# psweens/VAN-GAN

Hardware: AMD Instinct MI355X
Metric: train Mvoxels/s (VanGan.train_step, 128^3 bf16) (higher is better)
Workload: dtype bf16; 1 GPU; VanGan.train_step, 128x128x128 volumes, batch 1 per GPU (global 1), clDice on, disc noise+dropout on; parallelism=dp1

## Files before the change

### van_gan_amd/csrc/vg_conv_thin.hip

```cpp
#include "vg_conv_common.h"
#include <stdio.h>

static int vg_ablate_knob(const char* key) {
    const int v = vg_tune(key, 0);
#ifdef VG_DEBUG_ABLATE
    return v;
#else
    if (v != 0) { fprintf(stderr, "libvangan_hip: VG_%s=%d is a timing-ablation knob of a -DVG_DEBUG_ABLATE build; this library refuses it\n", key, v); return -1; }
    return 0;
#endif
}
#include "vg_dma_common.h"
#include <type_traits>
#include <algorithm>
#include <cstdio>

#ifndef VG_THIN_WPE
#define VG_THIN_WPE 2
#endif
#ifndef VG_THIN_PF2
#define VG_THIN_PF2 0
#endif
#ifndef VG_THIN_PD
#define VG_THIN_PD 1
// ... 547 lines not shown
        auto epilogue = [&](auto masked_tag, const int pn16) {
            constexpr bool MASKED = decltype(masked_tag)::value;
            const bool dw_ok = !MASKED || (od < p.OD && ow < p.OW);
            const int nrow = MASKED ? p.OH - oh0 : TH;
            typedef __attribute__((ext_vector_type(2))) unsigned u32x2;
            typedef __attribute__((ext_vector_type(4))) unsigned u32x4;
#pragma unroll
            for (int q = 0; q < NP; ++q) {
            T* const optr = (T*)p.out + obase + cst + 16 * q + pn16;
            const T* const rptr = RES ? (const T*)p.res + obase + co0 + 16 * q : nullptr;
            const float* const r1ptr = RES ? (const float*)p.res + (((size_t)(n * p.BD + od + p.ood) * p.BH + oh0 + p.ooh) * p.BW + ow + p.oow) : nullptr;
            f32x2 eb[2], ers[2], erb[2];
            if constexpr (NP == 1) { eb[0] = e_b[0][0]; eb[1] = e_b[0][1]; if (RES) { ers[0] = e_rs[0][0]; ers[1] = e_rs[0][1]; erb[0] = e_rb[0][0]; erb[1] = e_rb[0][1]; } }
            else {
                const float* eq = ebs + 4 * kg + 16 * q;
                if (BIAS) { const f32x4 t = *(const f32x4*)eq; eb[0] = (f32x2){t[0], t[1]}; eb[1] = (f32x2){t[2], t[3]}; }
                if (RES) {
                    const f32x4 t = *(const f32x4*)(eq + 16 * NP), u = *(const f32x4*)(eq + 32 * NP);
                    ers[0] = (f32x2){t[0], t[1]}; ers[1] = (f32x2){t[2], t[3]}; erb[0] = (f32x2){u[0], u[1]}; erb[1] = (f32x2){u[2], u[3]};
                }
            }
            bf16x4 bx[BSTAT ? 8 : 1];
            f32x2 b_sc[2], b_sf[2], b_rs[2], b_nm[2];
            if (BSTAT) {
                constexpr int CW = 16 * NP * PL;
                const float* bq = bsc + 4 * kg + 16 * q + pn16;
                const f32x4 c_sc = *(const f32x4*)bq, c_sf = *(const f32x4*)(bq + CW), c_rs = *(const f32x4*)(bq + 2 * CW), c_nm = *(const f32x4*)(bq + 3 * CW);
                b_sc[0] = (f32x2){c_sc[0], c_sc[1]}; b_sc[1] = (f32x2){c_sc[2], c_sc[3]}; b_sf[0] = (f32x2){c_sf[0], c_sf[1]}; b_sf[1] = (f32x2){c_sf[2], c_sf[3]};
                b_rs[0] = (f32x2){c_rs[0], c_rs[1]}; b_rs[1] = (f32x2){c_rs[2], c_rs[3]};
                b_nm[0] = (f32x2){c_nm[0], c_nm[1]}; b_nm[1] = (f32x2){c_nm[2], c_nm[3]};
                auto fold = [&](int qq, int nn) { int i = qq - p.bs_pad; i = i < 0 ? -i : i; i = i >= nn ? 2 * nn - 2 - i : i; return min(max(i, 0), nn - 1); };
                const int XH = p.bs_H >> b_sh[q], XW = p.bs_W >> b_sh[q];
                const int id = fold(od + p.ood, p.bs_D) >> b_sh[q], iw = fold(ow + p.oow, p.bs_W) >> b_sh[q];
                const T* xcol = b_x[q] + ((size_t)id * XH * XW + iw) * b_cs[q];
#pragma unroll
                for (int j = 0; j < 8; ++j) {
                    if constexpr (NP == 1) bx[j] = bxp[j];
                    else {
                        const int ih = fold(oh0 + j + p.ooh, p.bs_H) >> b_sh[q];
                        bx[j] = *(const __attribute__((address_space(1))) bf16x4*)(uintptr_t)(xcol + (size_t)ih * XW * b_cs[q]);
                    }
                }
            }
            constexpr int RRN = NP == 1 ? 8 : 4;
            bf16x4 rr[RES ? 8 : 1];
#pragma unroll
            for (int jp = 0; jp < 8; jp += 2) {
                if constexpr (RES) {
                    if (jp % RRN == 0) {
#pragma unroll
                        for (int j = jp; j < jp + RRN; ++j) {
                            const bool ok = !MASKED || (dw_ok && j < nrow);
                            if (NP == 1 && p.res1) {
                                const float xv = ld_global(ok ? r1ptr + (size_t)j * p.BW : r1ptr);
                                rr[j] = __builtin_bit_cast(bf16x4, (u32x2){__float_as_uint(xv), 0u});
                            } else
                            rr[j] = *(const __attribute__((address_space(1))) bf16x4*)(uintptr_t)(ok ? rptr + j * rowpitch : rptr);
                        }
                    }
                }
                bf16x4 pk[2];
#pragma unroll
                for (int e = 0; e < 2; ++e) {
                    const int j = jp + e;
                    const bool ok = !MASKED || (dw_ok && j < nrow);
                    f32x2 v0 = {acc[q][j][0], acc[q][j][1]}, v1 = {acc[q][j][2], acc[q][j][3]};
                    if (BIAS) { v0 += eb[0]; v1 += eb[1]; }
                    if (RES) {
                        const bf16x4 r = rr[RES ? j : 0];
                        f32x2 r0 = {bf2f((bf16_t)r[0]), bf2f((bf16_t)r[1])}, r1 = {bf2f((bf16_t)r[2]), bf2f((bf16_t)r[3])};
                        if (NP == 1 && p.res1) { const float xv = __uint_as_float(__builtin_bit_cast(u32x2, r)[0]); r0 = (f32x2){xv, xv}; r1 = r0; }
                        v0 += r0 * ers[0] + erb[0]; v1 += r1 * ers[1] + erb[1];
                    }
                    pk[e] = (bf16x4){(short)f2bf(v0[0]), (short)f2bf(v0[1]), (short)f2bf(v1[0]), (short)f2bf(v1[1])};
                    if (STATS) {
                        f32x2 q0 = {bf2f((bf16_t)pk[e][0]), bf2f((bf16_t)pk[e][1])}, q1 = {bf2f((bf16_t)pk[e][2]), bf2f((bf16_t)pk[e][3])};
                        if (MASKED && !ok) { q0 = (f32x2){0.f, 0.f}; q1 = q0; }
                        f32x2 a0 = {s1[q][0], s1[q][1]}, a1 = {s1[q][2], s1[q][3]}, c0 = {s2[q][0], s2[q][1]}, c1 = {s2[q][2], s2[q][3]};
                        a0 += q0; a1 += q1; c0 += q0 * q0; c1 += q1 * q1;
                        s1[q][0] = a0[0]; s1[q][1] = a0[1]; s1[q][2] = a1[0]; s1[q][3] = a1[1]; s2[q][0] = c0[0]; s2[q][1] = c0[1]; s2[q][2] = c1[0]; s2[q][3] = c1[1];
                    }
                    if (BSTAT) {
                        f32x2 q0 = {bf2f((bf16_t)pk[e][0]), bf2f((bf16_t)pk[e][1])}, q1 = {bf2f((bf16_t)pk[e][2]), bf2f((bf16_t)pk[e][3])};
                        if (MASKED && !ok) { q0 = (f32x2){0.f, 0.f}; q1 = q0; }
                        const bf16x4 xr = bx[BSTAT ? j : 0];
                        const f32x2 x0 = {bf2f((bf16_t)xr[0]), bf2f((bf16_t)xr[1])}, x1 = {bf2f((bf16_t)xr[2]), bf2f((bf16_t)xr[3])};
                        const f32x2 pre0 = x0 * b_sc[0] + b_sf[0], pre1 = x1 * b_sc[1] + b_sf[1];
                        const f32x2 d0 = {pre0[0] > 0.f ? 1.f : b_slope, pre0[1] > 0.f ? 1.f : b_slope};
                        const f32x2 d1 = {pre1[0] > 0.f ? 1.f : b_slope, pre1[1] > 0.f ? 1.f : b_slope};
                        const f32x2 dn0 = q0 * d0, dn1 = q1 * d1;
                        const f32x2 xh0 = x0 * b_rs[0] + b_nm[0], xh1 = x1 * b_rs[1] + b_nm[1];
                        f32x2 a0 = {s1[q][0], s1[q][1]}, a1 = {s1[q][2], s1[q][3]}, c0 = {s2[q][0], s2[q][1]}, c1 = {s2[q][2], s2[q][3]};
                        a0 += dn0; a1 += dn1; c0 += dn0 * xh0; c1 += dn1 * xh1;
                        s1[q][0] = a0[0]; s1[q][1] = a0[1]; s1[q][2] = a1[0]; s1[q][3] = a1[1]; s2[q][0] = c0[0]; s2[q][1] = c0[1]; s2[q][2] = c1[0]; s2[q][3] = c1[1];
                    }
                }
                const u32x2 wa = __builtin_bit_cast(u32x2, pk[0]), wb2 = __builtin_bit_cast(u32x2, pk[1]);
                const u32x2 x0 = __builtin_amdgcn_permlane16_swap(wa[0], wb2[0], false, false);
                const u32x2 x1 = __builtin_amdgcn_permlane16_swap(wa[1], wb2[1], false, false);
                const u32x4 outv = {x0[0], x1[0], x0[1], x1[1]};
                const int j = jp + jodd;
                if (!MASKED || (dw_ok && j < nrow)) *(u32x4*)(optr + j * rowpitch) = outv;
                if constexpr (BSTAT && PL > 1) { __builtin_amdgcn_sched_barrier(0); bxn[jp] = bx_row(jp); bxn[jp + 1] = bx_row(jp + 1); __builtin_amdgcn_sched_barrier(0); }
            }
            }
        };
        if constexpr (PL == 1) { if (full) epilogue(std::false_type{}, 0); else epilogue(std::true_type{}, 0); }
        else {
            if (it) lds_only_barrier();
            if constexpr (BSTAT) {
                if (it == 0) {
                    bx_prepare(0, od0, oh0, ow0);
#pragma unroll
                    for (int j = 0; j < 8; ++j) bxn[j] = bx_row(j);
                }
            }
            if (!(p.dbg & 16) || it == 0) {
            thin_issue<MODE>(g, utab, tabat(od0, oh0, ow0), n, 0, tid, raw);
            thin_commit<MODE>(g, halo, scs, utab, tabat(od0, oh0, ow0), 0, tid, raw);
            }
#pragma unroll 1
            for (int pn = 0; pn < PL; ++pn) {
                const int use = it * PL + pn;
                if (use == 0) asm volatile("s_waitcnt vmcnt(0)" ::: "memory");
                lds_only_barrier();
                if (pn + 1 < PL || more) dma_weights(pn + 1 < PL ? pn + 1 : 0, (use + 1) & 1);
#pragma unroll
                for (int j = 0; j < 8; ++j) acc[0][j] = (f32x4){0.f, 0.f, 0.f, 0.f};
                if (!(p.dbg & 4)) mfma_panel(wlds + (use & 1) * WBUF + wbase);
                __builtin_amdgcn_s_waitcnt(0x0F70);
                asm volatile("" ::: "memory");
                if constexpr (BSTAT) {
#pragma unroll
                    for (int j = 0; j < 8; ++j) asm volatile("v_mov_b64 %0, %1" : "=&v"(bxp[j]) : "v"(bxn[j]));
                    if (pn + 1 < PL) bx_prepare(16 * (pn + 1), od0, oh0, ow0); else if (more) bx_prepare(0, ti_d * TD, ti_h * TH, ti_w * TW);
                }
                if (full) epilogue(std::false_type{}, 16 * pn); else epilogue(std::true_type{}, 16 * pn);
                if constexpr (BSTAT) {
#pragma unroll
                    for (int r = 0; r < 4; ++r) {
                        const float a = s1[0][r], b = s2[0][r];
#pragma unroll
                        for (int q = 0; q + 1 < PL; ++q) { s1[q][r] = s1[q + 1][r]; s2[q][r] = s2[q + 1][r]; }
                        s1[PL - 1][r] = a; s2[PL - 1][r] = b;
                    }
                }
            }
        }
    }
    if constexpr (PL > 1) asm volatile("s_waitcnt vmcnt(0)" ::: "memory");
    if ((STATS || BSTAT) && p.sums) {
#pragma unroll
        for (int q = 0; q < NP * PL; ++q)
#pragma unroll
            for (int r = 0; r < 4; ++r) {
                float a = s1[q][r], b = s2[q][r];
#pragma unroll
                for (int o = 1; o < 16; o <<= 1) { a += __shfl_xor(a, o); b += __shfl_xor(b, o); }
                if (li == 0) { atomicAdd(&stat[(16 * q + 4 * kg + r) * 2], a); atomicAdd(&stat[(16 * q + 4 * kg + r) * 2 + 1], b); }
            }
        __syncthreads();
        if (tid < 32 * NP * PL) {
            const int co = cop + (tid >> 1);
            const int stripe = blockIdx.x & (VG_STRIPES - 1);
            if (co < p.Cout) atomicAdd(&p.sums[(((size_t)stripe * gridDim.z + n) * p.Cout + co) * 2 + (tid & 1)], stat[tid]);
        }
        if constexpr (STATS && (NP == 2 || !RES)) { if (p.fin.ticket) vg_fin_tail(p.fin, p.sums, gridDim.z, p.Cout, gridDim.x * gridDim.y * gridDim.z, (int*)stat); }
    }
}

int vg_conv_thin_lds_bytes(const GatherIn& g, int np, int pl, bool up, bool wdma) {
    const int AL = (g.tiles_h * TH + 2) + (g.tiles_w * TW + 2) + (g.tiles_d * TD + 2);
    int head = HALO + (32 + 32 * np * pl + 64 * np * pl + (np > 1 ? 48 * np : 0) + 32) * 4 + (2 * HH * HW * 2 + 2 * AL) * 4;
    if (pl > 1 || wdma) return head + 1024 + 2 * 15 * 1024;
    if (up) {
        head += (g.tiles_h * (TH / 2) + 2 + g.tiles_d * (TD / 2) + 2 + 2 * UPCOLS + 16) * 4;
        return head + 16 + std::max(16 * np * (KCPAD * 2 + 16), 4 * 16 * np * WRSU);
    }
    return head + 16 + 16 * np * (KCPAD * 2 + 16);
}

bool vg_conv_thin_ok(const vg_conv_desc* d, const GatherIn& g, const ConvOut& k, const ConvCls& q, int np) {
    if (!vg_tune("CONV_THIN", 1)) return false;
    if (d->f32 || d->noise || q.ncls != 1 || d->istr != 1 || d->ostr != 1 || d->CK != 16 || d->ntaps != 27 || d->wpack) return false;
    if ((d->c_src0 + d->c_src1) % 16 || (d->Cout % (16 * np)) || d->tanh_out || d->accumulate || d->out_f32) return false;
    if (g.lean != VG_STAGE_PLAIN && g.lean != VG_STAGE_RELU) return false;
    if (!g.planar || g.HW != HW || g.HH != HH || g.HD != HD || g.HWp != HW || g.HHp != HH || g.DS != DSB || g.PSB != PSB) return false;
    if ((1 << g.twl) != TW || (1 << g.thl) != TH || (1 << g.tdl) != TD) return false;
    if (d->res && (d->bias == nullptr)) return false;
    if (d->res_c1 && np != 1) return false;
    if (k.Ktot != k.nchunks * KCPAD) return false;
    for (int i = 0; i < 27; ++i)
        if (d->tap_d[i] - g.tmin_d > 2 || d->tap_h[i] - g.tmin_h > 2 || d->tap_w[i] - g.tmin_w > 2) return false;
    if (np > 1) {
        const long wgs = (long)g.tiles_d * g.tiles_h * g.tiles_w * (d->Cout / (16 * np)) * d->N;
        if (!vg_tune("CONV_THIN2", 1) || wgs < vg_tune("CONV_THIN2_MINWG", 96)) return false;
    }
    return true;
}

template <int MODE, bool BIAS, bool RES, bool STATS, bool BSTAT, int NP, int PL = 1, bool UP = false>
static int launch_thin_np(const GatherIn& g, const ConvOut& k, int lds, hipStream_t s) {
    static bool attr_set = false;
    if (!attr_set) {
        (void)hipFuncSetAttribute((const void*)conv_thin_kernel<MODE, BIAS, RES, STATS, BSTAT, NP, PL, UP>, hipFuncAttributeMaxDynamicSharedMemorySize, VG_LDS_LIMIT);
        attr_set = true;
    }
    int per_cu = 2;
    if (lds > 0 && VG_LDS_LIMIT / lds < per_cu) per_cu = VG_LDS_LIMIT / lds;
    if (per_cu < 1) per_cu = 1;
    const int tiles = g.tiles_d * g.tiles_h * g.tiles_w;
    const int ny = k.Cout / (16 * NP * PL);
    const int wg = vg_tune("CONV_THIN_WGS", 0) > 0 ? vg_tune("CONV_THIN_WGS", 0) : 256 * per_cu;
    int bx = wg / (ny * g.N); if (bx < 1) bx = 1; if (bx > tiles) bx = tiles;
    ConvOut k2 = k; k2.xw = 0; k2.dbg = PL > 1 ? vg_ablate_knob("THIN_DBG") : 0;
    if (k2.dbg < 0) return VG_EINVAL;
    if (vg_tune("CONV_THIN_XCD", 1) && bx >= 16 && tiles >= 4 * bx) { bx &= ~7; k2.xw = 1; }
    char name[96];
    snprintf(name, sizeof name, "%s<m%%d,b%%d,r%%d,s%%d%s%s%s>|walk%%d|ch%%d", NP == 2 ? "conv_thin2" : "conv_thin", BSTAT ? (k.bs_x1 ? ",bs2" : ",bs1") : "", PL > 1 ? ",pl" : "", UP ? ",up" : "");
    if (vg_dry(name, MODE, (int)BIAS, (int)RES, (int)STATS, tiles > bx ? 1 : 0, k.nchunks > 1 ? (k.wdma ? 2 : 1) : 0)) return VG_OK;
    const bool fin_here = STATS && k2.fin.ticket && k2.sums && ((NP == 2 && vg_tune("CONV_THIN2_FIN", 1)) || (NP == 1 && !RES && vg_tune("CONV_THIN1_FIN", 1)));
    if (!fin_here) k2.fin.ticket = nullptr;
    if constexpr (!UP) k2.nup = 0;
    hipLaunchKernelGGL((conv_thin_kernel<MODE, BIAS, RES, STATS, BSTAT, NP, PL, UP>), dim3(bx, ny, g.N), dim3(256), lds, s, g, k2);
    if (fin_here) vg_fin_done = true;
    return vg_check_launch();
}
template <int MODE, bool BIAS, bool RES, bool STATS, bool BSTAT = false>
static int launch_thin(const GatherIn& g, const ConvOut& k, int np, hipStream_t s) {
    if constexpr (BSTAT && MODE == VG_STAGE_PLAIN) {
        const int lds3 = vg_conv_thin_lds_bytes(g, 1, 3);
        if (np == 1 && k.Cout == 48 && k.nchunks == 1 && 2 * lds3 <= VG_LDS_LIMIT && vg_tune("CONV_THIN_PL", 1))
            return launch_thin_np<MODE, BIAS, RES, STATS, BSTAT, 1, 3>(g, k, lds3, s);
    }
    if constexpr (MODE == VG_STAGE_RELU && BIAS && !RES && !BSTAT) {
        if (k.nup > 0 && k.nup < k.nchunks && vg_tune("CONV_THIN_UP", 0)) {
            const int ldsu = vg_conv_thin_lds_bytes(g, np, 1, true);
            if (2 * ldsu <= VG_LDS_LIMIT) {
                if (np == 1) return launch_thin_np<MODE, BIAS, RES, STATS, BSTAT, 1, 1, true>(g, k, ldsu, s);
            }
        }
    }
    if constexpr (MODE == VG_STAGE_RELU && !BSTAT) {
        const int ldsw = vg_conv_thin_lds_bytes(g, 1, 1, false, true);
        if (np == 1 && k.nchunks > 1 && 2 * ldsw <= VG_LDS_LIMIT && vg_tune("CONV_THIN_WDMA", 1)) {
            ConvOut kw = k; kw.wdma = 1;
            return launch_thin_np<MODE, BIAS, RES, STATS, BSTAT, 1>(g, kw, ldsw, s);
        }
    }
    const int lds = vg_conv_thin_lds_bytes(g, np);
    if (lds > VG_LDS_LIMIT) return VG_ELDS;
    if constexpr (!BSTAT) { if (np == 2) return launch_thin_np<MODE, BIAS, RES, STATS, BSTAT, 2>(g, k, lds, s); }
    return np == 1 ? launch_thin_np<MODE, BIAS, RES, STATS, BSTAT, 1>(g, k, lds, s) : VG_EINVAL;
}

int vg_launch_conv_thin(const GatherIn& g, const ConvOut& k, int np, hipStream_t s, float* red, bool& did_stats) {
    const bool st = k.sums != nullptr;
    if (g.lean == VG_STAGE_PLAIN) {
        if (np == 1 && red && k.bs_x0 && !k.bs_ml && k.bs_sc && k.bias == nullptr && k.res == nullptr && !st && (k.bs_c0 % 16) == 0 && (k.bs_c0 == k.Cout || k.bs_x1)
            && k.OD == k.BD && k.OH == k.BH && k.OW == k.BW && !k.ood && !k.ooh && !k.oow && vg_tune("CONV_BSTAT", 1)) {
            ConvOut k2 = k; k2.sums = red;
            const int rc = launch_thin<VG_STAGE_PLAIN, false, false, false, true>(g, k2, np, s);
            did_stats = rc == VG_OK && !vg_dry_on();
            return rc;
        }
        if (k.bias == nullptr && k.res == nullptr && !st) return launch_thin<VG_STAGE_PLAIN, false, false, false>(g, k, np, s);
        if (k.bias != nullptr && k.res == nullptr) return st ? launch_thin<VG_STAGE_PLAIN, true, false, true>(g, k, np, s)
                                                             : launch_thin<VG_STAGE_PLAIN, true, false, false>(g, k, np, s);
        return 1;
    }
    if (k.bias == nullptr) return 1;
    if (k.res != nullptr) return st ? launch_thin<VG_STAGE_RELU, true, true, true>(g, k, np, s) : launch_thin<VG_STAGE_RELU, true, true, false>(g, k, np, s);
    return st ? launch_thin<VG_STAGE_RELU, true, false, true>(g, k, np, s) : launch_thin<VG_STAGE_RELU, true, false, false>(g, k, np, s);
}

__global__ void pack_up_weights_kernel(const float* __restrict__ w, int Cin, int Cout, int nup, bf16_t* __restrict__ out) {
    const int total = nup * 4 * Cout * KUP;
    for (int i = blockIdx.x * blockDim.x + threadIdx.x; i < total; i += gridDim.x * blockDim.x) {
        int t = i;
        const int kk = t % KUP; t /= KUP;
        const int co = t % Cout; t /= Cout;
        const int cls = t & 3, chunk = t >> 2;
        const int t12 = kk >> 4, cl = kk & 15, cdh = t12 / 3, cw = t12 - cdh * 3;
        const int cd = cdh >> 1, ch = cdh & 1, pd = cls >> 1, ph = cls & 1;
        const int d0 = pd == 0 ? (cd == 0 ? 0 : 1) : (cd == 0 ? 0 : 2), d1 = pd == 0 ? (cd == 0 ? 0 : 2) : (cd == 0 ? 1 : 2);
        const int h0 = ph == 0 ? (ch == 0 ? 0 : 1) : (ch == 0 ? 0 : 2), h1 = ph == 0 ? (ch == 0 ? 0 : 2) : (ch == 0 ? 1 : 2);
        const int ci = chunk * 16 + cl;
        float a = 0.f;
        for (int a_ = d0; a_ <= d1; ++a_)
            for (int b_ = h0; b_ <= h1; ++b_) a += w[((size_t)((a_ * 3 + b_) * 3 + cw) * Cin + ci) * Cout + co];
        out[i] = f2bf(a);
    }
}
extern "C" int vg_pack_up_weights(const float* w, int Cin, int Cout, int c_up, void* out, vg_stream_t stream) {
    vg_begin();
    if (!w || !out || Cin < 16 || Cout < 1 || c_up < 16 || (c_up % 16) || c_up > Cin) return VG_EINVAL;
    const int nup = c_up / 16, total = nup * 4 * Cout * KUP;
    hipLaunchKernelGGL(pack_up_weights_kernel, dim3(std::min((total + 255) / 256, 2048)), dim3(256), 0, (hipStream_t)stream, w, Cin, Cout, nup, (bf16_t*)out);
    return vg_check_launch();
}

struct WgThin { const void* dy; float* part; float* dw; float* db; int Cin, nslab, dbg; unsigned* tickets; int ntickets, xw; };
namespace {
constexpr int WT_DYROW = TW * 32 + 128;
constexpr int WT_DYB = TD * TH * WT_DYROW;
constexpr int WT_SLAB = 28 * 256;
}

template <int MODE>
__global__ __launch_bounds__(256, 2) void wgrad_thin_kernel(const GatherIn g, const WgThin p) {
    typedef bf16_t T;
    extern __shared__ __attribute__((aligned(16))) char smem[];
    const int tid = threadIdx.x, lane = tid & 63, wave = __builtin_amdgcn_readfirstlane(tid >> 6);
    const int chunk = blockIdx.y, n = blockIdx.z;
    const int PSBs = g.PSB;
    char* halo = smem;
    float* scs = (float*)(smem + 2 * PSBs);
    int* utab = (int*)(scs + 32);
    constexpr int NCOLS = HH * HW * 2;
    int* xtab = utab + 2 * NCOLS;
    const int NHt = g.tiles_h * TH + 2, NWt = g.tiles_w * TW + 2, NDt = g.tiles_d * TD + 2;
    char* dyt = (char*)(xtab + 2 * (NHt + NWt + NDt));
    dyt = (char*)(((size_t)dyt + 15) & ~(size_t)15);
    build_column_table(g, utab, tid);
    stage_scale_shift(g, scs, n, chunk, tid);
    thin_axis_tables(g, xtab, NHt, NWt, NDt, tid);
    if (blockIdx.x == 0 && blockIdx.y == 0 && blockIdx.z == 0 && tid < p.ntickets) p.tickets[tid] = 0u;
    __syncthreads();
    auto tabat = [&](int od0_, int oh0_, int ow0_) { return ThinTab{xtab, NHt + NWt + NDt, NHt, NWt, od0_, oh0_, ow0_}; };
    const int gq = lane >> 4, q = (lane >> 2) & 3, pp = lane & 3;
    const int wq = 8 * (gq & 1) + q, yq = gq >> 1;
    const int abase = (pp >> 1) * PSBs + ((wave * HH + yq) * HW + wq) * UNIT + (pp & 1) * 8;
    const int bbase = (wave * TH + yq) * WT_DYROW + wq * 32 + (wq >> 3) * 128 + pp * 8;
    f32x4 acc[28];
#pragma unroll
    for (int t = 0; t < 28; ++t) acc[t] = (f32x4){0.f, 0.f, 0.f, 0.f};
    bf16x8 ones;
    { const short o = (short)f2bf(1.f); ones = (bf16x8){o, o, o, o, o, o, o, o}; }
    typedef __attribute__((ext_vector_type(4))) short s16x4;
    typedef __attribute__((address_space(3))) s16x4 lds_s4;
    const int tiles_per_n = g.tiles_d * g.tiles_h * g.tiles_w;
    const T* dyn = (const T*)p.dy + (size_t)n * g.D * g.H * g.W * 16;
    Raw8<T> raw[3][HD / 2];
    f32x4 dv[4];
    auto origin = [&](int tile, int& od0, int& oh0, int& ow0) {
        const int ti_w = tile % g.tiles_w, t2 = tile / g.tiles_w, ti_h = t2 % g.tiles_h, ti_d = t2 / g.tiles_h;
        od0 = ti_d * TD; oh0 = ti_h * TH; ow0 = ti_w * TW;
    };
    auto issue = [&](int od0, int oh0, int ow0) {
        thin_issue<MODE>(g, utab, tabat(od0, oh0, ow0), n, chunk, tid, raw);
#pragma unroll
        for (int i = 0; i < 4; ++i) {
            const int u = tid + 256 * i, vox = u >> 1, w = vox & 15, y = (vox >> 4) & 7, z = vox >> 7;
            const bool ok = od0 + z < g.D && oh0 + y < g.H && ow0 + w < g.W;
            const T* src = dyn + (((size_t)min(od0 + z, g.D - 1) * g.H + min(oh0 + y, g.H - 1)) * g.W + min(ow0 + w, g.W - 1)) * 16 + (u & 1) * 8;
            dv[i] = *(const __attribute__((address_space(1))) f32x4*)(uintptr_t)src;
            if (!ok) dv[i] = (f32x4){0.f, 0.f, 0.f, 0.f};
        }
    };
    int t0 = blockIdx.x, tstep = gridDim.x, tend = tiles_per_n;
    if (p.xw) {
        const int sl = (tiles_per_n + 7) >> 3, xcd = blockIdx.x & 7;
        t0 = xcd * sl + ((int)blockIdx.x >> 3); tstep = gridDim.x >> 3; tend = min(tiles_per_n, (xcd + 1) * sl);
    }
    int od0, oh0, ow0;
    if (t0 < tend) { origin(t0, od0, oh0, ow0); issue(od0, oh0, ow0); }
    unsigned long long c_wait0 = 0, c_commit = 0, c_wait1 = 0, c_k = 0, t_a = 0, t_b = 0;
    for (int tile = t0; tile < tend; tile += tstep) {
        if (p.dbg & 8) t_a = __builtin_amdgcn_s_memtime();
        __syncthreads();
        if (p.dbg & 8) { t_b = __builtin_amdgcn_s_memtime(); c_wait0 += t_b - t_a; }
        if (!(p.dbg & 2)) thin_commit<MODE>(g, halo, scs, utab, tabat(od0, oh0, ow0), chunk, tid, raw);
#pragma unroll
        for (int i = 0; i < 4; ++i) {
            const int u = tid + 256 * i, vox = u >> 1, w = vox & 15;
            *(f32x4*)(dyt + (vox >> 4) * WT_DYROW + w * 32 + (w >> 3) * 128 + (u & 1) * 16) = dv[i];
        }
        if (p.dbg & 8) { asm volatile("s_waitcnt lgkmcnt(0)" ::: "memory"); t_a = __builtin_amdgcn_s_memtime(); c_commit += t_a - t_b; }
        __syncthreads();
        if (p.dbg & 8) { t_b = __builtin_amdgcn_s_memtime(); c_wait1 += t_b - t_a; }
        if (!(p.dbg & 4) && tile + tstep < tend) { origin(tile + tstep, od0, oh0, ow0); issue(od0, oh0, ow0); }
        if (p.dbg & 1) continue;
        constexpr int WG_ = 6, NG_ = 4 * 27 / WG_;
        bf16x8 afr[2][WG_], bfr[2];
        auto load_b = [&](int s) {
            const s16x4 bl = __builtin_amdgcn_ds_read_tr16_b64_v4i16((lds_s4*)(dyt + bbase + s * 2 * WT_DYROW));
            const s16x4 bh = __builtin_amdgcn_ds_read_tr16_b64_v4i16((lds_s4*)(dyt + bbase + s * 2 * WT_DYROW + 128));
            bfr[s & 1] = (bf16x8){bl[0], bl[1], bl[2], bl[3], bh[0], bh[1], bh[2], bh[3]};
        };
        auto load_group = [&](int i, int set) {
#pragma unroll
            for (int k = 0; k < WG_; ++k) {
                const int e = i * WG_ + k, s = e / 27, t = e - 27 * s;
                if (t == 0) load_b(s);
                const int o = abase + (t / 9) * DSB + ((t / 3) % 3 + 2 * s) * ROWB + (t % 3) * UNIT;
                const s16x4 al = __builtin_amdgcn_ds_read_tr16_b64_v4i16((lds_s4*)(halo + o));
                const s16x4 ah = __builtin_amdgcn_ds_read_tr16_b64_v4i16((lds_s4*)(halo + o + 4 * UNIT));
                afr[set][k] = (bf16x8){al[0], al[1], al[2], al[3], ah[0], ah[1], ah[2], ah[3]};
            }
        };
        load_group(0, 0);
#pragma unroll
        for (int i = 0; i < NG_; ++i) {
            if (i + 1 < NG_) load_group(i + 1, (i + 1) & 1);
            __builtin_amdgcn_sched_barrier(0);
#pragma unroll
            for (int k = 0; k < WG_; ++k) {
                const int e = i * WG_ + k, s = e / 27, t = e - 27 * s;
                acc[t] = VG_MFMA16(afr[i & 1][k], bfr[s & 1], acc[t]);
                if (t == 26) acc[27] = VG_MFMA16(ones, bfr[s & 1], acc[27]);
            }
            __builtin_amdgcn_sched_barrier(0);
        }
        if (p.dbg & 8) { t_a = __builtin_amdgcn_s_memtime(); c_k += t_a - t_b; }
    }
    if ((p.dbg & 8) && tid == 0) {
        unsigned long long* o = (unsigned long long*)(p.tickets + 4096) + ((size_t)(blockIdx.z * gridDim.y + blockIdx.y) * gridDim.x + blockIdx.x) * 4;
        o[0] = c_wait0; o[1] = c_commit; o[2] = c_wait1; o[3] = c_k;
    }
    float* red = (float*)halo;
    for (int w = 0; w < 4; ++w) {
        __syncthreads();
        if (wave == w) {
#pragma unroll
            for (int t = 0; t < 28; ++t)
#pragma unroll
                for (int e = 0; e < 4; ++e) {
                    float* r = red + (t * 4 + e) * 64 + lane;
                    *r = w == 0 ? acc[t][e] : *r + acc[t][e];
                }
        }
    }
    __syncthreads();
    float* slab = p.part + ((size_t)chunk * p.nslab + (size_t)n * gridDim.x + blockIdx.x) * WT_SLAB;
    for (int i = tid; i < 28 * 256; i += 256) {
        const int l = i & 63, e = (i >> 6) & 3, t = i >> 8;
        slab[t * 256 + (4 * (l >> 4) + e) * 16 + (l & 15)] = red[i];
    }
}

constexpr int WT_RG = 8;
__global__ __launch_bounds__(256) void wgrad_thin_reduce_kernel(const float* part, int nslab, int Cin, float* dw, float* db, float* part2, unsigned* tickets) {
    __shared__ f32x4 sm[4][64];
    __shared__ int last;
    const int lane = threadIdx.x & 63, w = threadIdx.x >> 6, chunk = blockIdx.y, gr = blockIdx.z;
    const int j = (blockIdx.x * 64 + lane) * 4;
    const float* base = part + (size_t)chunk * nslab * WT_SLAB + j;
    f32x4 s = {0.f, 0.f, 0.f, 0.f};
    int b = 4 * gr + w;
    for (; b + 60 * WT_RG < nslab; b += 64 * WT_RG) {
        f32x4 v[16];
#pragma unroll
        for (int k = 0; k < 16; ++k) v[k] = *(const f32x4*)(base + (size_t)(b + 4 * WT_RG * k) * WT_SLAB);
#pragma unroll
        for (int k = 0; k < 16; ++k) s += v[k];
    }
    for (; b < nslab; b += 4 * WT_RG) s += *(const f32x4*)(base + (size_t)b * WT_SLAB);
    sm[w][lane] = s;
    __syncthreads();
    float* col = part2 + ((size_t)(chunk * 28 + blockIdx.x) * WT_RG) * 256;
    if (w == 0) {
        const f32x4 r = ((sm[0][lane] + sm[1][lane]) + sm[2][lane]) + sm[3][lane];
        float* o = col + gr * 256 + lane * 4;
#pragma unroll
        for (int k = 0; k < 4; ++k) __hip_atomic_store(o + k, r[k], __ATOMIC_RELAXED, __HIP_MEMORY_SCOPE_AGENT);
    }
    asm volatile("s_waitcnt vmcnt(0)" ::: "memory");
    __syncthreads();
    if (threadIdx.x == 0) {
        unsigned* tk = tickets + chunk * 28 + blockIdx.x;
        const unsigned old = __hip_atomic_fetch_add(tk, 1u, __ATOMIC_RELAXED, __HIP_MEMORY_SCOPE_AGENT);
        last = old == WT_RG - 1;
        if (last) __hip_atomic_store(tk, 0u, __ATOMIC_RELAXED, __HIP_MEMORY_SCOPE_AGENT);
    }
    __syncthreads();
    if (!last || w != 0) return;
    f32x4 r = {0.f, 0.f, 0.f, 0.f};
#pragma unroll
    for (int g2 = 0; g2 < WT_RG; ++g2)
#pragma unroll
        for (int k = 0; k < 4; ++k) r[k] += __hip_atomic_load(col + g2 * 256 + lane * 4 + k, __ATOMIC_RELAXED, __HIP_MEMORY_SCOPE_AGENT);
    const int t = j >> 8, ci = (j >> 4) & 15, co = j & 15;
    if (t < 27) {
        float* o = dw + ((size_t)t * Cin + 16 * chunk + ci) * 16 + co;
#pragma unroll
        for (int k = 0; k < 4; ++k) atomicAdd(o + k, r[k]);
    } else if (ci == 0 && chunk == 0 && db) {
#pragma unroll
        for (int k = 0; k < 4; ++k) atomicAdd(db + co + k, r[k]);
    }
}

int vg_wgrad_thin(const vg_conv_desc* d, const void* dy, int dy_f32, const int32_t* tap_idx_host, int T_total, float* dw, float* db,
                  float* scratch, int64_t scratch_bytes, hipStream_t s) {
    if (!vg_tune("WGRAD_THIN", 1) || d->f32 || dy_f32 || d->src_f32 || d->wpack || d->noise || d->nclass > 1) return 1;
    const int Cin = d->c_src0 + d->c_src1;
    if (d->ntaps != 27 || T_total != 27 || d->istr != 1 || d->Cout != 16 || (Cin % 16) || Cin < 16 || Cin > 64 || d->CK != 16) return 1;
    if (d->OD != d->D || d->OH != d->H || d->OW != d->W) return 1;
    if ((int64_t)d->D * d->H * d->W < vg_tune("WGRAD_THIN_MINVOX", 65536)) return 1;
    int tmin[3] = {d->tap_d[0], d->tap_h[0], d->tap_w[0]};
    for (int t = 0; t < 27; ++t)
        if (tap_idx_host[t] != t || d->tap_d[t] != tmin[0] + t / 9 || d->tap_h[t] != tmin[1] + (t / 3) % 3 || d->tap_w[t] != tmin[2] + t % 3) return 1;
    GatherIn g;
    if (fill_gather(d, g, 16, 512) != VG_OK) return 1;
    if (g.lean != VG_STAGE_PLAIN && g.lean != VG_STAGE_RELU) return 1;
    if (!g.planar || g.HW != HW || g.HH != HH || g.HD != HD || g.HWp != HW || g.HHp != HH || g.DS != DSB || g.PSB != PSB) return 1;
    g.PSB += 64; g.CS = g.PSB;
    if ((1 << g.twl) != TW || (1 << g.thl) != TH || (1 << g.tdl) != TD) return 1;
    const int AL = (g.tiles_h * TH + 2) + (g.tiles_w * TW + 2) + (g.tiles_d * TD + 2);
    const int lds = 2 * g.PSB + 32 * 4 + (2 * HH * HW * 2 + 2 * AL) * 4 + 16 + WT_DYB;
    if (lds > VG_LDS_LIMIT || 2 * g.PSB < WT_SLAB * 4) return 1;
    const int nchunks = Cin / 16, tiles = g.tiles_d * g.tiles_h * g.tiles_w;
    int bx = vg_tune("WGRAD_THIN_WGS", 512) / (nchunks * d->N);
    if (bx < 1) bx = 1; if (bx > tiles) bx = tiles;
    int xw = 0;
    if (vg_tune("WGRAD_THIN_XCD", 1) && bx >= 16 && tiles >= 4 * bx) { bx &= ~7; xw = 1; }
    const int nslab = bx * d->N;
    const int64_t slab_f = (int64_t)nchunks * nslab * WT_SLAB, part2_f = (int64_t)nchunks * 28 * WT_RG * 256;
    if (!scratch || (slab_f + part2_f + nchunks * 28 + 64 + 4096 + 8 * 4096) * 4 > scratch_bytes) return 1;
    if (vg_dry("wgrad_thin<m%d>|ch%d|walk%d", g.lean, nchunks > 1 ? 1 : 0, tiles > bx ? 1 : 0)) return VG_OK;
    float* part2 = scratch + slab_f;
    unsigned* tickets = (unsigned*)(part2 + part2_f);
    const int wt_dbg = vg_ablate_knob("WT_DBG");
    if (wt_dbg < 0) return VG_EINVAL;
    WgThin p = {dy, scratch, dw, db, Cin, nslab, wt_dbg, tickets, nchunks * 28, xw};
    const dim3 grid(bx, nchunks, d->N);
    if (g.lean == VG_STAGE_PLAIN) {
        static bool a0 = false;
        if (!a0) { (void)hipFuncSetAttribute((const void*)wgrad_thin_kernel<VG_STAGE_PLAIN>, hipFuncAttributeMaxDynamicSharedMemorySize, VG_LDS_LIMIT); a0 = true; }
        hipLaunchKernelGGL((wgrad_thin_kernel<VG_STAGE_PLAIN>), grid, dim3(256), lds, s, g, p);
    } else {
        static bool a1 = false;
        if (!a1) { (void)hipFuncSetAttribute((const void*)wgrad_thin_kernel<VG_STAGE_RELU>, hipFuncAttributeMaxDynamicSharedMemorySize, VG_LDS_LIMIT); a1 = true; }
        hipLaunchKernelGGL((wgrad_thin_kernel<VG_STAGE_RELU>), grid, dim3(256), lds, s, g, p);
    }
    hipLaunchKernelGGL(wgrad_thin_reduce_kernel, dim3(WT_SLAB / 256, nchunks, WT_RG), dim3(256), 0, s, (const float*)scratch, nslab, Cin, dw, db, part2, tickets);
    return vg_check_launch();
}
```

### van_gan_amd/csrc/vg_dma_common.h

```cpp
#pragma once
#include "vg_gather.h"

typedef __attribute__((address_space(3))) void lds_void_d;
typedef const __attribute__((address_space(1))) void glb_void_d;
typedef __attribute__((address_space(3))) bf16x4 lds_bf16x4_d;

struct MatK {
    const void* src0; const void* src1; int c0, c1, shift0;
    int N, D, H, W, Cin;
    const float* in_scale; const float* in_shift; int act;
    const bf16_t* noise; int npad;
    int pad_mode;
    int pmin_d, pmin_h, pmin_w;
    int Dp, Hp, Wp;
    int deint, WE, Wps;
    bf16_t* out;
};

void vg_launch_materialize(const MatK& m, hipStream_t s);

__device__ __forceinline__ int fast_div(int n, unsigned m) { return m ? (int)__umulhi((unsigned)n, m) : n; }

__device__ __forceinline__ void glds16(const char* sbase, int voff, unsigned lds_addr) {
    unsigned keep;
    asm volatile("s_mov_b32 %0, m0\n\ts_mov_b32 m0, %3\n\ts_nop 0\n\tglobal_load_lds_dwordx4 %1, %2\n\ts_mov_b32 m0, %0"
                 : "=&s"(keep) : "v"(voff), "s"(sbase), "s"(lds_addr) : "memory");
}

#define VG_VM1(i) "s_waitcnt vmcnt(" #i ")\n\ts_branch 2f\n\t"
#define VG_VM8(a, b, c, d, e, f, g, h) VG_VM1(a) VG_VM1(b) VG_VM1(c) VG_VM1(d) VG_VM1(e) VG_VM1(f) VG_VM1(g) VG_VM1(h)
__device__ __forceinline__ void wait_vmcnt(int n_) {
    const int n = __builtin_amdgcn_readfirstlane(n_);
    asm volatile(
        "s_min_u32 s42, %0, 40\n\t"
        "s_lshl_b32 s42, s42, 3\n\t"
        "s_getpc_b64 s[40:41]\n"
        "0:\n\t"
        "s_add_u32 s40, s40, s42\n\t"
        "s_addc_u32 s41, s41, 0\n\t"
        "s_add_u32 s40, s40, 1f-0b\n\t"
        "s_addc_u32 s41, s41, 0\n\t"
        "s_setpc_b64 s[40:41]\n"
        "1:\n\t"
        VG_VM8(0, 1, 2, 3, 4, 5, 6, 7) VG_VM8(8, 9, 10, 11, 12, 13, 14, 15) VG_VM8(16, 17, 18, 19, 20, 21, 22, 23)
        VG_VM8(24, 25, 26, 27, 28, 29, 30, 31) VG_VM8(32, 33, 34, 35, 36, 37, 38, 39) VG_VM1(40)
        "2:\n\t"
        : : "s"(n) : "s40", "s41", "s42", "scc", "memory");
}

__device__ __forceinline__ void vg_pack_dma_units(const float* __restrict__ w, const int* __restrict__ tap_idx, bf16_t* __restrict__ out, int Cin, int Cout,
                                  int ntaps, int transpose, int bn, int u0, int ustride) {
    const int NR = transpose ? Cin : Cout, C = transpose ? Cout : Cin;
    const int npl = C >> 4;
    const unsigned units = (unsigned)NR * (unsigned)npl * (unsigned)ntaps * 2u;
    const bool vec = transpose && (((uintptr_t)w & 15) == 0) && (Cout % 8) == 0;
    for (unsigned u = (unsigned)u0; u < units; u += (unsigned)ustride) {
        unsigned t = u;
        const int row = (int)(t % (unsigned)bn); t /= (unsigned)bn;
        const int half = (int)(t & 1u); t >>= 1;
        const int tap = (int)(t % (unsigned)ntaps); t /= (unsigned)ntaps;
        const int plane = (int)(t % (unsigned)npl); const int cob = (int)(t / (unsigned)npl);
        const int r = cob * bn + row, c0 = plane * 16 + half * 8, ts = tap_idx[tap];
        float v[8];
        if (vec) load8<float>(w + ((size_t)ts * Cin + r) * Cout + c0, v);
        else {
#pragma unroll
            for (int e = 0; e < 8; ++e)
                v[e] = transpose ? w[((size_t)ts * Cin + r) * Cout + c0 + e] : w[((size_t)ts * Cin + c0 + e) * Cout + r];
        }
        store8<bf16_t>(out + (size_t)u * 8, v);
    }
}
```

Baseline: 123.2 Mvoxels/s.

## Double-buffer dY tiles via direct global-to-LDS DMA in thin wgrad

The wgrad thin kernel now loads the dY tile straight into a double-buffered LDS region with global_load_lds_dwordx4, instead of staging it through registers and writing it to LDS after the barrier. Out-of-bounds voxels read from a zero scratch buffer. The LDS row padding is replaced by an XOR-style swizzle of the write positions. The A-fragment prefetch depth becomes a compile-time knob, defaulting to 8 sets of 2. The aim is to free VGPRs, drop the commit-phase LDS stores and overlap the dY fetch with compute, at the price of twice the dY LDS footprint and a vmcnt(0) wait before the barrier.

Result: no change. 123.9 Mvoxels/s (median of 6 runs) (+0.6%).

```diff
diff --git a/van_gan_amd/csrc/vg_conv_thin.hip b/van_gan_amd/csrc/vg_conv_thin.hip
--- a/van_gan_amd/csrc/vg_conv_thin.hip
+++ b/van_gan_amd/csrc/vg_conv_thin.hip
@@ -873,10 +873,17 @@
 
 struct WgThin { const void* dy; float* part; float* dw; float* db; int Cin, nslab, dbg; unsigned* tickets; int ntickets, xw; };
 namespace {
-constexpr int WT_DYROW = TW * 32 + 128;
+constexpr int WT_DYROW = TW * 32;
 constexpr int WT_DYB = TD * TH * WT_DYROW;
 constexpr int WT_SLAB = 28 * 256;
 }
+__device__ __attribute__((aligned(16))) unsigned wt_zero16[4];
+#ifndef VG_WT_WG
+#define VG_WT_WG 2
+#endif
+#ifndef VG_WT_SETS
+#define VG_WT_SETS 8
+#endif
 
 template <int MODE>
 __global__ __launch_bounds__(256, 2) void wgrad_thin_kernel(const GatherIn g, const WgThin p) {
@@ -885,14 +892,14 @@
     const int tid = threadIdx.x, lane = tid & 63, wave = __builtin_amdgcn_readfirstlane(tid >> 6);
     const int chunk = blockIdx.y, n = blockIdx.z;
     const int PSBs = g.PSB;
-    char* halo = smem;
-    float* scs = (float*)(smem + 2 * PSBs);
+    char* dyt = smem;
+    char* halo = smem + 2 * WT_DYB;
+    float* scs = (float*)(halo + 2 * PSBs);
     int* utab = (int*)(scs + 32);
     constexpr int NCOLS = HH * HW * 2;
     int* xtab = utab + 2 * NCOLS;
     const int NHt = g.tiles_h * TH + 2, NWt = g.tiles_w * TW + 2, NDt = g.tiles_d * TD + 2;
-    char* dyt = (char*)(xtab + 2 * (NHt + NWt + NDt));
-    dyt = (char*)(((size_t)dyt + 15) & ~(size_t)15);
+    const unsigned dyt_a = (unsigned)(uintptr_t)(lds_void_d*)dyt;
     build_column_table(g, utab, tid);
     stage_scale_shift(g, scs, n, chunk, tid);
     thin_axis_tables(g, xtab, NHt, NWt, NDt, tid);
@@ -902,7 +909,8 @@
     const int gq = lane >> 4, q = (lane >> 2) & 3, pp = lane & 3;
     const int wq = 8 * (gq & 1) + q, yq = gq >> 1;
     const int abase = (pp >> 1) * PSBs + ((wave * HH + yq) * HW + wq) * UNIT + (pp & 1) * 8;
-    const int bbase = (wave * TH + yq) * WT_DYROW + wq * 32 + (wq >> 3) * 128 + pp * 8;
+    const int bbase = (wave * TH + yq) * WT_DYROW + q * 32 + pp * 8;
+    const int bb0 = bbase + (gq & 1) * 384, bb1 = bbase + 128 + (gq & 1) * 128;
     f32x4 acc[28];
 #pragma unroll
     for (int t = 0; t < 28; ++t) acc[t] = (f32x4){0.f, 0.f, 0.f, 0.f};
@@ -913,21 +921,22 @@
     const int tiles_per_n = g.tiles_d * g.tiles_h * g.tiles_w;
     const T* dyn = (const T*)p.dy + (size_t)n * g.D * g.H * g.W * 16;
     Raw8<T> raw[3][HD / 2];
-    f32x4 dv[4];
     auto origin = [&](int tile, int& od0, int& oh0, int& ow0) {
         const int ti_w = tile % g.tiles_w, t2 = tile / g.tiles_w, ti_h = t2 % g.tiles_h, ti_d = t2 / g.tiles_h;
         od0 = ti_d * TD; oh0 = ti_h * TH; ow0 = ti_w * TW;
     };
-    auto issue = [&](int od0, int oh0, int ow0) {
+    auto issue = [&](int od0, int oh0, int ow0, int buf) {
+        const char* tb = (const char*)dyn + (((size_t)(od0 + wave) * g.H + oh0) * g.W + ow0) * 32;
+        int ln = lane;
+        asm volatile("" : "+v"(ln));
+#pragma unroll
+        for (int k = 0; k < 4; ++k) {
+            const int u = 64 * k + ln, y = u >> 5, sb = (u >> 3) & 3, w = ((sb ^ (sb >> 1)) << 2) + ((u >> 1) & 3);
+            const bool ok = od0 + wave < g.D && oh0 + y < g.H && ow0 + w < g.W;
+            const char* src = tb + (unsigned)((y * g.W + w) * 32 + (u & 1) * 16);
+            glds16a(ok ? (const void*)src : (const void*)wt_zero16, dyt_a + buf * WT_DYB + (4 * wave + k) * 1024);
+        }
         thin_issue<MODE>(g, utab, tabat(od0, oh0, ow0), n, chunk, tid, raw);
-#pragma unroll
-        for (int i = 0; i < 4; ++i) {
-            const int u = tid + 256 * i, vox = u >> 1, w = vox & 15, y = (vox >> 4) & 7, z = vox >> 7;
-            const bool ok = od0 + z < g.D && oh0 + y < g.H && ow0 + w < g.W;
-            const T* src = dyn + (((size_t)min(od0 + z, g.D - 1) * g.H + min(oh0 + y, g.H - 1)) * g.W + min(ow0 + w, g.W - 1)) * 16 + (u & 1) * 8;
-            dv[i] = *(const __attribute__((address_space(1))) f32x4*)(uintptr_t)src;
-            if (!ok) dv[i] = (f32x4){0.f, 0.f, 0.f, 0.f};
-        }
     };
     int t0 = blockIdx.x, tstep = gridDim.x, tend = tiles_per_n;
     if (p.xw) {
@@ -935,28 +944,27 @@
         t0 = xcd * sl + ((int)blockIdx.x >> 3); tstep = gridDim.x >> 3; tend = min(tiles_per_n, (xcd + 1) * sl);
     }
     int od0, oh0, ow0;
-    if (t0 < tend) { origin(t0, od0, oh0, ow0); issue(od0, oh0, ow0); }
+    int cur = 0;
+    if (t0 < tend) { origin(t0, od0, oh0, ow0); issue(od0, oh0, ow0, 0); }
     unsigned long long c_wait0 = 0, c_commit = 0, c_wait1 = 0, c_k = 0, t_a = 0, t_b = 0;
-    for (int tile = t0; tile < tend; tile += tstep) {
+    for (int tile = t0; tile < tend; tile += tstep, cur ^= 1) {
         if (p.dbg & 8) t_a = __builtin_amdgcn_s_memtime();
         __syncthreads();
         if (p.dbg & 8) { t_b = __builtin_amdgcn_s_memtime(); c_wait0 += t_b - t_a; }
         if (!(p.dbg & 2)) thin_commit<MODE>(g, halo, scs, utab, tabat(od0, oh0, ow0), chunk, tid, raw);
-#pragma unroll
-        for (int i = 0; i < 4; ++i) {
-            const int u = tid + 256 * i, vox = u >> 1, w = vox & 15;
-            *(f32x4*)(dyt + (vox >> 4) * WT_DYROW + w * 32 + (w >> 3) * 128 + (u & 1) * 16) = dv[i];
-        }
         if (p.dbg & 8) { asm volatile("s_waitcnt lgkmcnt(0)" ::: "memory"); t_a = __builtin_amdgcn_s_memtime(); c_commit += t_a - t_b; }
+        asm volatile("s_waitcnt vmcnt(0)" ::: "memory");
         __syncthreads();
         if (p.dbg & 8) { t_b = __builtin_amdgcn_s_memtime(); c_wait1 += t_b - t_a; }
-        if (!(p.dbg & 4) && tile + tstep < tend) { origin(tile + tstep, od0, oh0, ow0); issue(od0, oh0, ow0); }
+        if (!(p.dbg & 4) && tile + tstep < tend) { origin(tile + tstep, od0, oh0, ow0); issue(od0, oh0, ow0, cur ^ 1); }
         if (p.dbg & 1) continue;
-        constexpr int WG_ = 6, NG_ = 4 * 27 / WG_;
-        bf16x8 afr[2][WG_], bfr[2];
+        constexpr int WG_ = VG_WT_WG, NS_ = VG_WT_SETS, NG_ = 4 * 27 / WG_;
+        static_assert(NG_ * WG_ == 4 * 27 && NS_ >= 2 && (NS_ - 1) * WG_ <= 27, "groups tile the 108 products; dY fragments are read at most one K-step ahead");
+        bf16x8 afr[NS_][WG_], bfr[2];
+        char* dyc = dyt + cur * WT_DYB;
         auto load_b = [&](int s) {
-            const s16x4 bl = __builtin_amdgcn_ds_read_tr16_b64_v4i16((lds_s4*)(dyt + bbase + s * 2 * WT_DYROW));
-            const s16x4 bh = __builtin_amdgcn_ds_read_tr16_b64_v4i16((lds_s4*)(dyt + bbase + s * 2 * WT_DYROW + 128));
+            const s16x4 bl = __builtin_amdgcn_ds_read_tr16_b64_v4i16((lds_s4*)(dyc + bb0 + s * 2 * WT_DYROW));
+            const s16x4 bh = __builtin_amdgcn_ds_read_tr16_b64_v4i16((lds_s4*)(dyc + bb1 + s * 2 * WT_DYROW));
             bfr[s & 1] = (bf16x8){bl[0], bl[1], bl[2], bl[3], bh[0], bh[1], bh[2], bh[3]};
         };
         auto load_group = [&](int i, int set) {
@@ -970,15 +978,16 @@
                 afr[set][k] = (bf16x8){al[0], al[1], al[2], al[3], ah[0], ah[1], ah[2], ah[3]};
             }
         };
-        load_group(0, 0);
+#pragma unroll
+        for (int i = 0; i < NS_ - 1; ++i) load_group(i, i);
 #pragma unroll
         for (int i = 0; i < NG_; ++i) {
-            if (i + 1 < NG_) load_group(i + 1, (i + 1) & 1);
+            if (i + NS_ - 1 < NG_) load_group(i + NS_ - 1, (i + NS_ - 1) % NS_);
             __builtin_amdgcn_sched_barrier(0);
 #pragma unroll
             for (int k = 0; k < WG_; ++k) {
                 const int e = i * WG_ + k, s = e / 27, t = e - 27 * s;
-                acc[t] = VG_MFMA16(afr[i & 1][k], bfr[s & 1], acc[t]);
+                acc[t] = VG_MFMA16(afr[i % NS_][k], bfr[s & 1], acc[t]);
                 if (t == 26) acc[27] = VG_MFMA16(ones, bfr[s & 1], acc[27]);
             }
             __builtin_amdgcn_sched_barrier(0);
@@ -1079,7 +1088,7 @@
     g.PSB += 64; g.CS = g.PSB;
     if ((1 << g.twl) != TW || (1 << g.thl) != TH || (1 << g.tdl) != TD) return 1;
     const int AL = (g.tiles_h * TH + 2) + (g.tiles_w * TW + 2) + (g.tiles_d * TD + 2);
-    const int lds = 2 * g.PSB + 32 * 4 + (2 * HH * HW * 2 + 2 * AL) * 4 + 16 + WT_DYB;
+    const int lds = 2 * WT_DYB + 2 * g.PSB + 32 * 4 + (2 * HH * HW * 2 + 2 * AL) * 4;
     if (lds > VG_LDS_LIMIT || 2 * g.PSB < WT_SLAB * 4) return 1;
     const int nchunks = Cin / 16, tiles = g.tiles_d * g.tiles_h * g.tiles_w;
     int bx = vg_tune("WGRAD_THIN_WGS", 512) / (nchunks * d->N);
diff --git a/van_gan_amd/csrc/vg_dma_common.h b/van_gan_amd/csrc/vg_dma_common.h
--- a/van_gan_amd/csrc/vg_dma_common.h
+++ b/van_gan_amd/csrc/vg_dma_common.h
@@ -25,6 +25,12 @@
     unsigned keep;
     asm volatile("s_mov_b32 %0, m0\n\ts_mov_b32 m0, %3\n\ts_nop 0\n\tglobal_load_lds_dwordx4 %1, %2\n\ts_mov_b32 m0, %0"
                  : "=&s"(keep) : "v"(voff), "s"(sbase), "s"(lds_addr) : "memory");
+}
+
+__device__ __forceinline__ void glds16a(const void* src, unsigned lds_addr) {
+    unsigned keep;
+    asm volatile("s_mov_b32 %0, m0\n\ts_mov_b32 m0, %2\n\ts_nop 0\n\tglobal_load_lds_dwordx4 %1, off\n\ts_mov_b32 m0, %0"
+                 : "=&s"(keep) : "v"(src), "s"(lds_addr) : "memory");
 }
 
 #define VG_VM1(i) "s_waitcnt vmcnt(" #i ")\n\ts_branch 2f\n\t"
```
